# tuna2134/sbv2-api

Measured on NVIDIA B200. Metric: audio-sec/sec, higher is better.
Workload: dtype f16 operands / f32 accumulate on tcgen05 (decoder, flow; text encoder with two-term fp16 splits); f32 elsewhere

## Files before the change

sbv2-api_b200/csrc/flow_attention_tc.cu:

```cuda
#include <cuda_fp16.h>
#include <math_constants.h>

#include "kernels.h"

namespace sbv2 {
namespace {

constexpr int QT = 128, KT = 128, D = 96, DP = D / 8, RP = 16;
constexpr uint32_t TILE_BYTES = DP * KT * 16;
constexpr uint32_t P_BYTES = (KT / 8) * QT * 16;
constexpr uint32_t PREL_BYTES = (RP / 8) * QT * 16;
constexpr uint32_t REL_BYTES = DP * RP * 16;
constexpr int TM_O = 0, TM_SREL = 96, TM_S = 128 , TM_COLS = 512;
constexpr int NKV = 3;
constexpr int NSM_WARPS = 8;

__device__ __forceinline__ uint32_t smem_u32(const void* p) { return (uint32_t)__cvta_generic_to_shared(p); }
__device__ __forceinline__ void mbar_init(uint32_t bar, uint32_t count) {
  asm volatile("mbarrier.init.shared::cta.b64 [%0], %1;" ::"r"(bar), "r"(count));
}
__device__ __forceinline__ void mbar_expect_tx(uint32_t bar, uint32_t bytes) {
  asm volatile("mbarrier.arrive.expect_tx.shared::cta.b64 _, [%0], %1;" ::"r"(bar), "r"(bytes) : "memory");
}
__device__ __forceinline__ void mbar_arrive(uint32_t bar) {
  asm volatile("mbarrier.arrive.shared::cta.b64 _, [%0];" ::"r"(bar) : "memory");
}
__device__ __forceinline__ void mbar_wait(uint32_t bar, uint32_t parity) {
  asm volatile(
      "{\n"
      ".reg .pred P1;\n"
      "LAB_WAIT:\n"
      "mbarrier.try_wait.parity.shared::cta.b64 P1, [%0], %1, %2;\n"
      "@P1 bra DONE;\n"
      "bra LAB_WAIT;\n"
      "DONE:\n"
      "}\n" ::"r"(bar),
      "r"(parity), "r"(0x989680u)
      : "memory");
}
__device__ __forceinline__ void bulk_g2s(uint32_t dst, const void* src, uint32_t bytes, uint32_t bar) {
  asm volatile("cp.async.bulk.shared::cluster.global.mbarrier::complete_tx::bytes [%0], [%1], %2, [%3];" ::"r"(dst), "l"(src),
               "r"(bytes), "r"(bar)
               : "memory");
}
__device__ __forceinline__ void tc_fence_before() { asm volatile("tcgen05.fence::before_thread_sync;" ::: "memory"); }
__device__ __forceinline__ void tc_fence_after() { asm volatile("tcgen05.fence::after_thread_sync;" ::: "memory"); }
__device__ __forceinline__ void tc_commit(uint32_t bar) {
  asm volatile("tcgen05.commit.cta_group::1.mbarrier::arrive::one.shared::cluster.b64 [%0];" ::"r"(bar) : "memory");
}
__device__ __forceinline__ void tc_mma_f16(uint32_t tmem_d, uint64_t adesc, uint64_t bdesc, uint32_t idesc, uint32_t accumulate) {
  asm volatile(
      "{\n"
      ".reg .pred p;\n"
      "setp.ne.b32 p, %4, 0;\n"
      "tcgen05.mma.cta_group::1.kind::f16 [%0], %1, %2, %3, p;\n"
      "}\n" ::"r"(tmem_d),
      "l"(adesc), "l"(bdesc), "r"(idesc), "r"(accumulate)
      : "memory");
}
__device__ __forceinline__ void tc_ld32(uint32_t taddr, uint32_t* v) {
  asm volatile(
      "tcgen05.ld.sync.aligned.32x32b.x32.b32 "
      "{%0,%1,%2,%3,%4,%5,%6,%7,%8,%9,%10,%11,%12,%13,%14,%15,%16,%17,%18,%19,%20,%21,%22,%23,%24,%25,%26,%27,%28,%29,%30,%31}, [%32];"
      : "=r"(v[0]), "=r"(v[1]), "=r"(v[2]), "=r"(v[3]), "=r"(v[4]), "=r"(v[5]), "=r"(v[6]), "=r"(v[7]), "=r"(v[8]), "=r"(v[9]),
        "=r"(v[10]), "=r"(v[11]), "=r"(v[12]), "=r"(v[13]), "=r"(v[14]), "=r"(v[15]), "=r"(v[16]), "=r"(v[17]), "=r"(v[18]),
        "=r"(v[19]), "=r"(v[20]), "=r"(v[21]), "=r"(v[22]), "=r"(v[23]), "=r"(v[24]), "=r"(v[25]), "=r"(v[26]), "=r"(v[27]),
        "=r"(v[28]), "=r"(v[29]), "=r"(v[30]), "=r"(v[31])
      : "r"(taddr)
      : "memory");
}
__device__ __forceinline__ void tc_ld16(uint32_t taddr, uint32_t* v) {
  asm volatile(
      "tcgen05.ld.sync.aligned.32x32b.x16.b32 {%0,%1,%2,%3,%4,%5,%6,%7,%8,%9,%10,%11,%12,%13,%14,%15}, [%16];"
      : "=r"(v[0]), "=r"(v[1]), "=r"(v[2]), "=r"(v[3]), "=r"(v[4]), "=r"(v[5]), "=r"(v[6]), "=r"(v[7]), "=r"(v[8]), "=r"(v[9]),
        "=r"(v[10]), "=r"(v[11]), "=r"(v[12]), "=r"(v[13]), "=r"(v[14]), "=r"(v[15])
      : "r"(taddr)
      : "memory");
}
__device__ __forceinline__ void tc_wait_ld() { asm volatile("tcgen05.wait::ld.sync.aligned;" ::: "memory"); }
__device__ __forceinline__ uint32_t elect_one_sync() {
  uint32_t pred = 0;
  asm volatile(
      "{\n"
      ".reg .b32 %%rx;\n"
      ".reg .pred %%px;\n"
      "elect.sync %%rx|%%px, %1;\n"
      "@%%px mov.s32 %0, 1;\n"
      "}\n"
      : "+r"(pred)
      : "r"(0xffffffffu));
  return pred;
}
__device__ __forceinline__ float ex2_approx(float x) {
  float y;
  asm("ex2.approx.ftz.f32 %0, %1;" : "=f"(y) : "f"(x));
  return y;
}
__device__ __forceinline__ uint64_t make_desc(uint32_t saddr, uint32_t lbo_bytes, uint32_t sbo_bytes) {
  return (uint64_t)((saddr >> 4) & 0x3FFF) | ((uint64_t)((lbo_bytes >> 4) & 0x3FFF) << 16) | ((uint64_t)((sbo_bytes >> 4) & 0x3FFF) << 32) |
         ((uint64_t)1 << 46);
}
constexpr uint32_t idesc_f16(int n, int b_mn_major) {
  return (1u << 4) | ((uint32_t)b_mn_major << 16) | ((uint32_t)(n >> 3) << 17) | ((uint32_t)(128 >> 4) << 24);
}

#define ATRACE(ev, i)                                                                                   \
  do {                                                                                                   \
    if (trace != nullptr && blockIdx.x == 0 && blockIdx.y == 0 && blockIdx.z == 0 && (i) < 64) trace[(i) * 8 + (ev)] = clock64(); \
  } while (0)

__global__ void __launch_bounds__(288, 1) flow_attention_tc_kernel(__half* out, const __half* qkv, const __half* rel_k_p,
                                                                    const __half* rel_v_p, int heads, int window, PlanarSegs s,
                                                                    long long* trace) {
  extern __shared__ __align__(128) uint8_t smem[];
  const int warp = __shfl_sync(0xffffffffu, (int)(threadIdx.x >> 5), 0), lane = threadIdx.x & 31;
  const int b = s.order ? s.order[blockIdx.z] : (int)blockIdx.z, h = blockIdx.y;
  const int len = s.len[b];
  const int q0 = blockIdx.x * QT;
  if (q0 >= len) return;
  const long long pbase = s.pstart[b];
  const int n_kt = (len + KT - 1) / KT;

  const uint32_t sQ = smem_u32(smem);
  const uint32_t sK0 = sQ + TILE_BYTES;
  const uint32_t sV0 = sK0 + NKV * TILE_BYTES;
  const uint32_t sP = sV0 + NKV * TILE_BYTES;
  const uint32_t sPrel = sP + P_BYTES;
  const uint32_t sEk = sPrel + PREL_BYTES;
  const uint32_t sEv = sEk + REL_BYTES;
  const uint32_t sBar = sEv + REL_BYTES;
  const uint32_t bar_q = sBar, bar_kv = sBar + 8 , bar_kvfree = sBar + 40 , bar_s = sBar + 72 ,
                 bar_sfree = sBar + 88 , bar_p = sBar + 104, bar_pfree = sBar + 112, bar_done = sBar + 120;
  const uint32_t tmem_slot = sBar + 128;
  float* ml_x = reinterpret_cast<float*>(smem + (sBar - sQ) + 256);
  volatile uint32_t* tmem_slot_ptr = reinterpret_cast<volatile uint32_t*>(smem + (tmem_slot - sQ));

  if (threadIdx.x == 0) {
    mbar_init(bar_q, 1);
    for (int i = 0; i < NKV; ++i) {
      mbar_init(bar_kv + 8 * i, 1);
      mbar_init(bar_kvfree + 8 * i, 1);
    }
    mbar_init(bar_s, 1);
    mbar_init(bar_s + 8, 1);
    mbar_init(bar_sfree, 32 * NSM_WARPS);
    mbar_init(bar_sfree + 8, 32 * NSM_WARPS);
    mbar_init(bar_p, 32 * NSM_WARPS);
    mbar_init(bar_pfree, 1);
    mbar_init(bar_done, 1);
    asm volatile("fence.mbarrier_init.release.cluster;" ::: "memory");
  }
  if (warp == NSM_WARPS) {
    asm volatile("tcgen05.alloc.cta_group::1.sync.aligned.shared::cta.b32 [%0], %1;" ::"r"(tmem_slot), "r"((uint32_t)TM_COLS) : "memory");
    asm volatile("tcgen05.relinquish_alloc_permit.cta_group::1.sync.aligned;" ::: "memory");
  }
  if (threadIdx.x < 128) {
    const uint4 z = make_uint4(0, 0, 0, 0);
    *reinterpret_cast<uint4*>(smem + (sPrel - sQ) + threadIdx.x * 16) = z;
    *reinterpret_cast<uint4*>(smem + (sPrel - sQ) + QT * 16 + threadIdx.x * 16) = z;
  }
  asm volatile("fence.proxy.async.shared::cta;" ::: "memory");
  tc_fence_before();
  __syncthreads();
  tc_fence_after();
  const uint32_t tmem = *tmem_slot_ptr;
  pdl_launch_dependents();
  pdl_wait();

  const int q_plane0 = h * DP, k_plane0 = heads * DP + h * DP, v_plane0 = 2 * heads * DP + h * DP;
  const int n_tiles_total = 2 * n_kt;

  if (warp == NSM_WARPS) {
    auto load_tile = [&](int i) {
      const int buf = i % NKV;
      const uint32_t par = ((i / NKV) & 1) ^ 1;
      const int kt = i < n_kt ? i : i - n_kt;
      const bool with_v = i >= n_kt;
      const long long row0 = pbase + (long long)kt * KT;
      mbar_wait(bar_kvfree + 8 * buf, par);
      if (lane == 0) mbar_expect_tx(bar_kv + 8 * buf, with_v ? 2 * TILE_BYTES : TILE_BYTES);
      __syncwarp();
      if (lane < DP) {
        bulk_g2s(sK0 + buf * TILE_BYTES + lane * KT * 16, qkv + (size_t)(k_plane0 + lane) * s.plane_stride + row0 * 8, KT * 16,
                 bar_kv + 8 * buf);
      } else if (lane < 2 * DP && with_v) {
        const int pl = lane - DP;
        bulk_g2s(sV0 + buf * TILE_BYTES + pl * KT * 16, qkv + (size_t)(v_plane0 + pl) * s.plane_stride + row0 * 8, KT * 16,
                 bar_kv + 8 * buf);
      }
      __syncwarp();
    };
    if (elect_one_sync()) {
      mbar_expect_tx(bar_q, TILE_BYTES + 2 * REL_BYTES);
      for (int pl = 0; pl < DP; ++pl)
        bulk_g2s(sQ + pl * QT * 16, qkv + (size_t)(q_plane0 + pl) * s.plane_stride + (pbase + q0) * 8, QT * 16, bar_q);
      bulk_g2s(sEk, rel_k_p, REL_BYTES, bar_q);
      bulk_g2s(sEv, rel_v_p, REL_BYTES, bar_q);
    }
    __syncwarp();
    for (int i = 0; i < NKV && i < n_tiles_total; ++i) load_tile(i);
    mbar_wait(bar_q, 0);
    tc_fence_after();
    const uint64_t dq = make_desc(sQ, QT * 16, 128);
    const uint64_t dek = make_desc(sEk, RP * 16, 128);
    const uint64_t dp = make_desc(sP, QT * 16, 128);
    const uint64_t dprel = make_desc(sPrel, QT * 16, 128);
    const uint64_t dev = make_desc(sEv, 128, RP * 16);
    constexpr uint32_t ID_S = idesc_f16(KT, 0), ID_REL = idesc_f16(RP, 0), ID_O = idesc_f16(D, 1);
    if (elect_one_sync()) {
      for (int k = 0; k < D / 16; ++k)
        tc_mma_f16(tmem + TM_SREL, dq + (uint64_t)(k * 2 * QT), dek + (uint64_t)(k * 2 * RP), ID_REL, k > 0 ? 1u : 0u);
    }
    __syncwarp();
    auto issue_s = [&](int i) {
      const int sb = i & 1, kb = i % NKV;
      mbar_wait(bar_kv + 8 * kb, (i / NKV) & 1);
      if (lane == 0) ATRACE(0, i);
      mbar_wait(bar_sfree + 8 * sb, ((i >> 1) & 1) ^ 1);
      tc_fence_after();
      if (lane == 0) ATRACE(1, i);
      const uint64_t dk = make_desc(sK0 + kb * TILE_BYTES, KT * 16, 128);
      if (elect_one_sync()) {
        for (int k = 0; k < D / 16; ++k)
          tc_mma_f16(tmem + TM_S + sb * KT, dq + (uint64_t)(k * 2 * QT), dk + (uint64_t)(k * 2 * KT), ID_S, k > 0 ? 1u : 0u);
        tc_commit(bar_s + 8 * sb);
        if (i < n_kt) tc_commit(bar_kvfree + 8 * kb);
      }
      __syncwarp();
    };
    issue_s(0);
    for (int i = 0; i < n_tiles_total; ++i) {
      const int kb = i % NKV;
      if (i + 1 < n_tiles_total) issue_s(i + 1);
      if (i >= n_kt) {
        const int j = i - n_kt;
        mbar_wait(bar_p, j & 1);
        tc_fence_after();
        if (lane == 0) ATRACE(2, i);
        const uint64_t dv = make_desc(sV0 + kb * TILE_BYTES, 128, KT * 16);
        if (elect_one_sync()) {
          for (int k = 0; k < KT / 16; ++k)
            tc_mma_f16(tmem + TM_O, dp + (uint64_t)(k * 2 * QT), dv + (uint64_t)(k * 16), ID_O, (j > 0 || k > 0) ? 1u : 0u);
          tc_commit(bar_pfree);
          tc_commit(bar_kvfree + 8 * kb);
        }
        __syncwarp();
      }
      if (i + NKV < n_tiles_total) load_tile(i + NKV);
      if (lane == 0) ATRACE(3, i);
    }
    if (elect_one_sync()) {
      tc_mma_f16(tmem + TM_O, dprel, dev, ID_O, 1u);
      tc_commit(bar_done);
    }
    __syncwarp();
  } else {
    const int quarter = warp & 3, half = warp >> 2;
    const int row = quarter * 32 + lane;
    const int qi = q0 + row;
    const uint32_t lane_addr = tmem + ((uint32_t)(quarter * 32) << 16);
    const float c_scale = 1.4426950408889634f / sqrtf((float)D);
    float srel[9];
    {
      mbar_wait(bar_s, 0);
      tc_fence_after();
      uint32_t v[16];
      tc_ld16(lane_addr + TM_SREL, v);
      tc_wait_ld();
#pragma unroll
      for (int r = 0; r < 9; ++r) srel[r] = __uint_as_float(v[r]) * c_scale;
    }
    float m2 = -CUDART_INF_F, l = 0.f, mb = 0.f;
    uint8_t* prow = smem + (sP - sQ) + row * 16;
    uint8_t* prel_row = smem + (sPrel - sQ) + row * 16;
    auto pass_a = [&](const float* x, float c) {
      float mx = x[0];
#pragma unroll
      for (int e = 1; e < 32; ++e) mx = fmaxf(mx, x[e]);
      m2 = fmaxf(m2, mx * c);
    };
    auto pass_b_store = [&](const float* x, float c, int c32, float* pv) {
      float sum = 0.f;
#pragma unroll
      for (int e = 0; e < 32; ++e) {
        pv[e] = ex2_approx(fmaf(x[e], c, -mb));
        sum += pv[e];
      }
      l += sum;
#pragma unroll
      for (int q = 0; q < 4; ++q) {
        uint4 u;
        __half2* uh = reinterpret_cast<__half2*>(&u);
#pragma unroll
        for (int e = 0; e < 4; ++e) uh[e] = __floats2half2_rn(pv[q * 8 + 2 * e], pv[q * 8 + 2 * e + 1]);
        *reinterpret_cast<uint4*>(prow + (size_t)(c32 * 4 + q) * QT * 16) = u;
      }
    };
    for (int i = 0; i < n_tiles_total; ++i) {
      const bool pass_b = i >= n_kt;
      const int kt = pass_b ? i - n_kt : i;
      const int k0 = kt * KT;
      const int buf = i & 1;
      if (i > 0) {
        mbar_wait(bar_s + 8 * buf, (i >> 1) & 1);
        tc_fence_after();
      }
      if (threadIdx.x == 0) ATRACE(4, i);
      if (i == n_kt) {
        ml_x[(half * QT + row) * 2] = m2;
        asm volatile("bar.sync 1, %0;" ::"r"(32 * NSM_WARPS) : "memory");
        mb = fmaxf(m2, ml_x[((half ^ 1) * QT + row) * 2]);
      }
      if (pass_b && kt > 0) mbar_wait(bar_pfree, (kt - 1) & 1);
      if (threadIdx.x == 0) ATRACE(5, i);
#pragma unroll 1
      for (int cc = 0; cc < KT / 64; ++cc) {
        const int c = half * (KT / 64) + cc;
        const int kc0 = k0 + c * 32;
        if (kc0 >= len) {
          if (pass_b) {
            const uint4 z = make_uint4(0, 0, 0, 0);
#pragma unroll
            for (int q = 0; q < 4; ++q) *reinterpret_cast<uint4*>(prow + (size_t)(c * 4 + q) * QT * 16) = z;
          }
          continue;
        }
        uint32_t v[32];
        tc_ld32(lane_addr + TM_S + buf * KT + c * 32, v);
        tc_wait_ld();
        float* x = reinterpret_cast<float*>(v);
        const int j0 = kc0 - qi + 4;
        const bool band = j0 <= 8 && j0 + 31 >= 0;
        const bool tail = kc0 + 32 > len;
        if (!__any_sync(0xffffffffu, band) && !tail) {
          if (!pass_b) {
            pass_a(x, c_scale);
          } else {
            float pv[32];
            pass_b_store(x, c_scale, c, pv);
          }
          continue;
        }
#pragma unroll
        for (int e = 0; e < 32; ++e) {
          const int r = j0 + e;
          float add = 0.f;
#pragma unroll
          for (int rr = 0; rr < 9; ++rr) add = (r == rr) ? srel[rr] : add;
          x[e] = (kc0 + e < len) ? fmaf(x[e], c_scale, add) : -CUDART_INF_F;
        }
        if (!pass_b) {
          pass_a(x, 1.0f);
        } else {
          float pv[32];
          pass_b_store(x, 1.0f, c, pv);
#pragma unroll
          for (int rr = 0; rr < 9; ++rr) {
            const int e = rr - j0;
            float val = 0.f;
#pragma unroll
            for (int ee = 0; ee < 32; ++ee) val = (e == ee) ? pv[ee] : val;
            if (e >= 0 && e < 32) *reinterpret_cast<__half*>(prel_row + (size_t)(rr >> 3) * QT * 16 + (rr & 7) * 2) = __float2half_rn(val);
          }
        }
      }
      if (threadIdx.x == 0) ATRACE(6, i);
      tc_fence_before();
      mbar_arrive(bar_sfree + 8 * buf);
      if (pass_b) {
        asm volatile("fence.proxy.async.shared::cta;" ::: "memory");
        mbar_arrive(bar_p);
      }
    }
    ml_x[(half * QT + row) * 2 + 1] = l;
    asm volatile("bar.sync 1, %0;" ::"r"(32 * NSM_WARPS) : "memory");
    const float inv_l = 1.0f / (l + ml_x[((half ^ 1) * QT + row) * 2 + 1]);
    mbar_wait(bar_done, 0);
    tc_fence_after();
#pragma unroll 1
    for (int c = half * 2; c < (half == 0 ? 2 : D / 32); ++c) {
      uint32_t v[32];
      tc_ld32(lane_addr + TM_O + c * 32, v);
      tc_wait_ld();
      if (qi < len) {
#pragma unroll
        for (int q = 0; q < 4; ++q) {
          uint4 u;
          __half2* uh = reinterpret_cast<__half2*>(&u);
#pragma unroll
          for (int e = 0; e < 4; ++e)
            uh[e] = __floats2half2_rn(__uint_as_float(v[q * 8 + 2 * e]) * inv_l, __uint_as_float(v[q * 8 + 2 * e + 1]) * inv_l);
          *reinterpret_cast<uint4*>(out + (size_t)(h * DP + c * 4 + q) * s.plane_stride + (pbase + qi) * 8) = u;
        }
      }
    }
  }
  tc_fence_before();
  __syncthreads();
  if (warp == NSM_WARPS) {
    asm volatile("tcgen05.dealloc.cta_group::1.sync.aligned.b32 %0, %1;" ::"r"(tmem), "r"((uint32_t)TM_COLS) : "memory");
  }
}

}

std::vector<__half> pack_flow_rel_table(const float* table, int window, int head_dim) {
  const int R = 2 * window + 1;
  if (head_dim != D || R > RP) fail(SBV2_ERR_UNSUPPORTED, "tensor-core attention: head_dim must be 96 and window at most 7");
  std::vector<__half> pk(size_t(DP) * RP * 8, __float2half(0.f));
  for (int r = 0; r < R; ++r)
    for (int d = 0; d < D; ++d) pk[(size_t(d / 8) * RP + r) * 8 + d % 8] = __float2half_rn(table[size_t(r) * D + d]);
  return pk;
}

void launch_flow_attention_tc(const LaunchCtx& ctx, __half* ctx_out, const __half* qkv, const __half* rel_k_p, const __half* rel_v_p,
                              int heads, int head_dim, int window, const PlanarSegs& s, long long* trace) {
  if (s.n <= 0 || s.max_len <= 0) return;
  if (head_dim != D || window != 4) fail(SBV2_ERR_UNSUPPORTED, "tensor-core attention: head_dim must be 96 and window 4");
  const size_t smem = (1 + 2 * NKV) * TILE_BYTES + P_BYTES + PREL_BYTES + 2 * REL_BYTES + 256 + 2 * QT * 2 * 4;
  static PerDeviceOnce attr_once;
  attr_once.run([&] { CUDA_CHECK(cudaFuncSetAttribute(flow_attention_tc_kernel, cudaFuncAttributeMaxDynamicSharedMemorySize, (int)smem)); });
  dim3 grid((s.max_len + QT - 1) / QT, heads, s.n);
  launch_pdl(ctx.pdl, flow_attention_tc_kernel, grid, dim3(32 * (NSM_WARPS + 1)), smem, ctx.stream, ctx_out, qkv, rel_k_p, rel_v_p, heads, window, s,
             trace);
  ctx.count();
}

}

#ifdef SBV2_DEBUG_HOOKS
#include "model.h"
#include "umma_conv.h"
extern "C" int sbv2_debug_attn_trace(int T, int n_utt, int heads, long long* out_trace , float* out_ms) {
  using namespace sbv2;
  return guarded([&] {
    sbv2_model owner;
    owner.device = 0;
    CUDA_CHECK(cudaSetDevice(0));
    CUDA_CHECK(cudaStreamCreateWithFlags(&owner.stream, cudaStreamNonBlocking));
    LaunchCtx ctx = owner.ctx();
    DBuf meta, qkv, out, tr, rel;
    PinnedBuf pin;
    for (DBuf* b : {&meta, &qkv, &out, &tr, &rel}) b->stream = owner.stream;
    std::vector<int> ystart, ylen, muls{1};
    for (int i = 0; i < n_utt; ++i) {
      ystart.push_back(i * T);
      ylen.push_back(T);
    }
    BatchGeom bg = build_geoms(&owner, meta, pin, ystart, ylen, muls);
    const Geom& G = bg.g[0];
    const int C = heads * D;
    qkv.ensure(size_t(G.rows_tot) * 3 * C * 2);
    out.ensure(size_t(G.rows_tot) * C * 2);
    rel.ensure(2 * REL_BYTES);
    tr.ensure(64 * 8 * 8);
    CUDA_CHECK(cudaMemsetAsync(qkv.p, 0x11, size_t(G.rows_tot) * 3 * C * 2, owner.stream));
    CUDA_CHECK(cudaMemsetAsync(rel.p, 0, 2 * REL_BYTES, owner.stream));
    CUDA_CHECK(cudaMemsetAsync(tr.p, 0, 64 * 8 * 8, owner.stream));
    PlanarSegs ps;
    ps.start = bg.d_ystart;
    ps.pstart = G.d_pstart;
    ps.len = G.d_len;
    ps.n = n_utt;
    ps.max_len = T;
    ps.plane_stride = G.rows_tot * 8;
    const __half* rk = rel.as<__half>();
    const __half* rv = rk + REL_BYTES / 2;
    for (int i = 0; i < 2; ++i) launch_flow_attention_tc(ctx, out.as<__half>(), qkv.as<__half>(), rk, rv, heads, D, 4, ps, nullptr);
    cudaEvent_t e0, e1;
    CUDA_CHECK(cudaEventCreate(&e0));
    CUDA_CHECK(cudaEventCreate(&e1));
    CUDA_CHECK(cudaEventRecord(e0, owner.stream));
    for (int i = 0; i < 5; ++i) launch_flow_attention_tc(ctx, out.as<__half>(), qkv.as<__half>(), rk, rv, heads, D, 4, ps, nullptr);
    CUDA_CHECK(cudaEventRecord(e1, owner.stream));
    launch_flow_attention_tc(ctx, out.as<__half>(), qkv.as<__half>(), rk, rv, heads, D, 4, ps, tr.as<long long>());
    CUDA_CHECK(cudaStreamSynchronize(owner.stream));
    float ms = 0.f;
    CUDA_CHECK(cudaEventElapsedTime(&ms, e0, e1));
    if (out_ms) *out_ms = ms / 5.f;
    cudaEventDestroy(e0);
    cudaEventDestroy(e1);
    if (out_trace) CUDA_CHECK(cudaMemcpy(out_trace, tr.p, 64 * 8 * 8, cudaMemcpyDeviceToHost));
  });
}
#endif
```

Baseline: 9317.

## Shrink flow attention smem/TMEM footprint to fit two CTAs per SM

Reworks the K/V pipeline from three combined K+V buffers into two generic tile slots that are filled with K, V, and then the Ev table in a single item sequence. The S accumulator drops from double to single buffering, and Ek is staged in the P region. TMEM allocation is halved to 256 columns and launch bounds allow two CTAs per SM. The S-free barrier now fires right after the last TMEM read, so the next QK^T can start earlier. The aim is to overlap work from two CTAs per SM on large grids; in exchange, per-CTA pipelining depth drops. Small grids launch with a padded shared-memory size so they still get one CTA per SM. A debug timing hook is also added.

```diff
diff --git a/sbv2-api_b200/csrc/flow_attention_tc.cu b/sbv2-api_b200/csrc/flow_attention_tc.cu
--- a/sbv2-api_b200/csrc/flow_attention_tc.cu
+++ b/sbv2-api_b200/csrc/flow_attention_tc.cu
@@ -11,9 +11,15 @@
 constexpr uint32_t P_BYTES = (KT / 8) * QT * 16;
 constexpr uint32_t PREL_BYTES = (RP / 8) * QT * 16;
 constexpr uint32_t REL_BYTES = DP * RP * 16;
-constexpr int TM_O = 0, TM_SREL = 96, TM_S = 128 , TM_COLS = 512;
-constexpr int NKV = 3;
+constexpr int TM_O = 0, TM_SREL = 96, TM_S = 128, TM_COLS = 256;
+constexpr int NSLOT = 2;
 constexpr int NSM_WARPS = 8;
+constexpr uint32_t BAR_BYTES = 256, ML_BYTES = 2 * QT * 2 * 4;
+constexpr uint32_t SMEM_BYTES = (1 + NSLOT) * TILE_BYTES + P_BYTES + PREL_BYTES + BAR_BYTES + ML_BYTES;
+static_assert(2 * (SMEM_BYTES + 1024) <= 228 * 1024, "two CTAs per SM must fit");
+constexpr uint32_t SOLO_SMEM_BYTES = 200 * 1024;
+static_assert(SOLO_SMEM_BYTES + 1024 > 114 * 1024 && SOLO_SMEM_BYTES + 1024 <= 227 * 1024, "one CTA per SM, within the opt-in limit");
+static_assert(REL_BYTES <= P_BYTES && REL_BYTES <= TILE_BYTES, "Ek / Ev are staged in the P region / a tile slot");
 
 __device__ __forceinline__ uint32_t smem_u32(const void* p) { return (uint32_t)__cvta_generic_to_shared(p); }
 __device__ __forceinline__ void mbar_init(uint32_t bar, uint32_t count) {
@@ -109,7 +115,7 @@
     if (trace != nullptr && blockIdx.x == 0 && blockIdx.y == 0 && blockIdx.z == 0 && (i) < 64) trace[(i) * 8 + (ev)] = clock64(); \
   } while (0)
 
-__global__ void __launch_bounds__(288, 1) flow_attention_tc_kernel(__half* out, const __half* qkv, const __half* rel_k_p,
+__global__ void __launch_bounds__(288, 2) flow_attention_tc_kernel(__half* out, const __half* qkv, const __half* rel_k_p,
                                                                     const __half* rel_v_p, int heads, int window, PlanarSegs s,
                                                                     long long* trace) {
   extern __shared__ __align__(128) uint8_t smem[];
@@ -122,29 +128,25 @@
   const int n_kt = (len + KT - 1) / KT;
 
   const uint32_t sQ = smem_u32(smem);
-  const uint32_t sK0 = sQ + TILE_BYTES;
-  const uint32_t sV0 = sK0 + NKV * TILE_BYTES;
-  const uint32_t sP = sV0 + NKV * TILE_BYTES;
+  const uint32_t sR0 = sQ + TILE_BYTES;
+  const uint32_t sP = sR0 + NSLOT * TILE_BYTES;
+  const uint32_t sEk = sP;
   const uint32_t sPrel = sP + P_BYTES;
-  const uint32_t sEk = sPrel + PREL_BYTES;
-  const uint32_t sEv = sEk + REL_BYTES;
-  const uint32_t sBar = sEv + REL_BYTES;
-  const uint32_t bar_q = sBar, bar_kv = sBar + 8 , bar_kvfree = sBar + 40 , bar_s = sBar + 72 ,
-                 bar_sfree = sBar + 88 , bar_p = sBar + 104, bar_pfree = sBar + 112, bar_done = sBar + 120;
-  const uint32_t tmem_slot = sBar + 128;
-  float* ml_x = reinterpret_cast<float*>(smem + (sBar - sQ) + 256);
+  const uint32_t sBar = sPrel + PREL_BYTES;
+  const uint32_t bar_q = sBar, bar_kv = sBar + 8 , bar_kvfree = sBar + 24 , bar_s = sBar + 40,
+                 bar_sfree = sBar + 48, bar_p = sBar + 56, bar_pfree = sBar + 64, bar_done = sBar + 72;
+  const uint32_t tmem_slot = sBar + 80;
+  float* ml_x = reinterpret_cast<float*>(smem + (sBar - sQ) + BAR_BYTES);
   volatile uint32_t* tmem_slot_ptr = reinterpret_cast<volatile uint32_t*>(smem + (tmem_slot - sQ));
 
   if (threadIdx.x == 0) {
     mbar_init(bar_q, 1);
-    for (int i = 0; i < NKV; ++i) {
+    for (int i = 0; i < NSLOT; ++i) {
       mbar_init(bar_kv + 8 * i, 1);
       mbar_init(bar_kvfree + 8 * i, 1);
     }
     mbar_init(bar_s, 1);
-    mbar_init(bar_s + 8, 1);
     mbar_init(bar_sfree, 32 * NSM_WARPS);
-    mbar_init(bar_sfree + 8, 32 * NSM_WARPS);
     mbar_init(bar_p, 32 * NSM_WARPS);
     mbar_init(bar_pfree, 1);
     mbar_init(bar_done, 1);
@@ -171,41 +173,47 @@
   const int n_tiles_total = 2 * n_kt;
 
   if (warp == NSM_WARPS) {
-    auto load_tile = [&](int i) {
-      const int buf = i % NKV;
-      const uint32_t par = ((i / NKV) & 1) ^ 1;
-      const int kt = i < n_kt ? i : i - n_kt;
-      const bool with_v = i >= n_kt;
+    const int n_items = 3 * n_kt + 1, t_ev = 3 * n_kt;
+    auto kitem = [&](int i) { return i < n_kt ? i : 2 * i - n_kt; };
+    int next_item = 0;
+    auto load_item = [&](int t) {
+      const int slot = t % NSLOT;
+      const uint32_t dst = sR0 + slot * TILE_BYTES, bar = bar_kv + 8 * slot;
+      mbar_wait(bar_kvfree + 8 * slot, ((t / NSLOT) & 1) ^ 1);
+      if (t == t_ev) {
+        if (elect_one_sync()) {
+          mbar_expect_tx(bar, REL_BYTES);
+          bulk_g2s(dst, rel_v_p, REL_BYTES, bar);
+        }
+        __syncwarp();
+        return;
+      }
+      const bool is_v = t >= n_kt && ((t - n_kt) & 1);
+      const int kt = t < n_kt ? t : (t - n_kt) >> 1;
       const long long row0 = pbase + (long long)kt * KT;
-      mbar_wait(bar_kvfree + 8 * buf, par);
-      if (lane == 0) mbar_expect_tx(bar_kv + 8 * buf, with_v ? 2 * TILE_BYTES : TILE_BYTES);
+      if (lane == 0) mbar_expect_tx(bar, TILE_BYTES);
       __syncwarp();
-      if (lane < DP) {
-        bulk_g2s(sK0 + buf * TILE_BYTES + lane * KT * 16, qkv + (size_t)(k_plane0 + lane) * s.plane_stride + row0 * 8, KT * 16,
-                 bar_kv + 8 * buf);
-      } else if (lane < 2 * DP && with_v) {
-        const int pl = lane - DP;
-        bulk_g2s(sV0 + buf * TILE_BYTES + pl * KT * 16, qkv + (size_t)(v_plane0 + pl) * s.plane_stride + row0 * 8, KT * 16,
-                 bar_kv + 8 * buf);
-      }
+      if (lane < DP)
+        bulk_g2s(dst + lane * KT * 16, qkv + (size_t)((is_v ? v_plane0 : k_plane0) + lane) * s.plane_stride + row0 * 8, KT * 16, bar);
       __syncwarp();
     };
+    auto load_upto = [&](int last) {
+      for (; next_item <= last && next_item < n_items; ++next_item) load_item(next_item);
+    };
     if (elect_one_sync()) {
-      mbar_expect_tx(bar_q, TILE_BYTES + 2 * REL_BYTES);
+      mbar_expect_tx(bar_q, TILE_BYTES + REL_BYTES);
       for (int pl = 0; pl < DP; ++pl)
         bulk_g2s(sQ + pl * QT * 16, qkv + (size_t)(q_plane0 + pl) * s.plane_stride + (pbase + q0) * 8, QT * 16, bar_q);
       bulk_g2s(sEk, rel_k_p, REL_BYTES, bar_q);
-      bulk_g2s(sEv, rel_v_p, REL_BYTES, bar_q);
     }
     __syncwarp();
-    for (int i = 0; i < NKV && i < n_tiles_total; ++i) load_tile(i);
+    load_upto(NSLOT - 1);
     mbar_wait(bar_q, 0);
     tc_fence_after();
     const uint64_t dq = make_desc(sQ, QT * 16, 128);
     const uint64_t dek = make_desc(sEk, RP * 16, 128);
     const uint64_t dp = make_desc(sP, QT * 16, 128);
     const uint64_t dprel = make_desc(sPrel, QT * 16, 128);
-    const uint64_t dev = make_desc(sEv, 128, RP * 16);
     constexpr uint32_t ID_S = idesc_f16(KT, 0), ID_REL = idesc_f16(RP, 0), ID_O = idesc_f16(D, 1);
     if (elect_one_sync()) {
       for (int k = 0; k < D / 16; ++k)
@@ -213,47 +221,53 @@
     }
     __syncwarp();
     auto issue_s = [&](int i) {
-      const int sb = i & 1, kb = i % NKV;
-      mbar_wait(bar_kv + 8 * kb, (i / NKV) & 1);
+      const int t = kitem(i), slot = t % NSLOT;
+      mbar_wait(bar_kv + 8 * slot, (t / NSLOT) & 1);
       if (lane == 0) ATRACE(0, i);
-      mbar_wait(bar_sfree + 8 * sb, ((i >> 1) & 1) ^ 1);
+      mbar_wait(bar_sfree, (i & 1) ^ 1);
       tc_fence_after();
       if (lane == 0) ATRACE(1, i);
-      const uint64_t dk = make_desc(sK0 + kb * TILE_BYTES, KT * 16, 128);
+      const uint64_t dk = make_desc(sR0 + slot * TILE_BYTES, KT * 16, 128);
       if (elect_one_sync()) {
         for (int k = 0; k < D / 16; ++k)
-          tc_mma_f16(tmem + TM_S + sb * KT, dq + (uint64_t)(k * 2 * QT), dk + (uint64_t)(k * 2 * KT), ID_S, k > 0 ? 1u : 0u);
-        tc_commit(bar_s + 8 * sb);
-        if (i < n_kt) tc_commit(bar_kvfree + 8 * kb);
+          tc_mma_f16(tmem + TM_S, dq + (uint64_t)(k * 2 * QT), dk + (uint64_t)(k * 2 * KT), ID_S, k > 0 ? 1u : 0u);
+        tc_commit(bar_s);
+        tc_commit(bar_kvfree + 8 * slot);
       }
       __syncwarp();
     };
     issue_s(0);
     for (int i = 0; i < n_tiles_total; ++i) {
-      const int kb = i % NKV;
       if (i + 1 < n_tiles_total) issue_s(i + 1);
       if (i >= n_kt) {
-        const int j = i - n_kt;
+        const int j = i - n_kt, t = kitem(i) + 1, slot = t % NSLOT;
         mbar_wait(bar_p, j & 1);
+        mbar_wait(bar_kv + 8 * slot, (t / NSLOT) & 1);
         tc_fence_after();
         if (lane == 0) ATRACE(2, i);
-        const uint64_t dv = make_desc(sV0 + kb * TILE_BYTES, 128, KT * 16);
+        const uint64_t dv = make_desc(sR0 + slot * TILE_BYTES, 128, KT * 16);
         if (elect_one_sync()) {
           for (int k = 0; k < KT / 16; ++k)
             tc_mma_f16(tmem + TM_O, dp + (uint64_t)(k * 2 * QT), dv + (uint64_t)(k * 16), ID_O, (j > 0 || k > 0) ? 1u : 0u);
           tc_commit(bar_pfree);
-          tc_commit(bar_kvfree + 8 * kb);
+          tc_commit(bar_kvfree + 8 * slot);
         }
         __syncwarp();
       }
-      if (i + NKV < n_tiles_total) load_tile(i + NKV);
+      load_upto((i + 1 < n_tiles_total ? kitem(i + 1) : t_ev - 1) + NSLOT);
       if (lane == 0) ATRACE(3, i);
     }
-    if (elect_one_sync()) {
-      tc_mma_f16(tmem + TM_O, dprel, dev, ID_O, 1u);
-      tc_commit(bar_done);
-    }
-    __syncwarp();
+    {
+      const int slot = t_ev % NSLOT;
+      mbar_wait(bar_kv + 8 * slot, (t_ev / NSLOT) & 1);
+      tc_fence_after();
+      const uint64_t dev = make_desc(sR0 + slot * TILE_BYTES, 128, RP * 16);
+      if (elect_one_sync()) {
+        tc_mma_f16(tmem + TM_O, dprel, dev, ID_O, 1u);
+        tc_commit(bar_done);
+      }
+      __syncwarp();
+    }
   } else {
     const int quarter = warp & 3, half = warp >> 2;
     const int row = quarter * 32 + lane;
@@ -300,9 +314,8 @@
       const bool pass_b = i >= n_kt;
       const int kt = pass_b ? i - n_kt : i;
       const int k0 = kt * KT;
-      const int buf = i & 1;
       if (i > 0) {
-        mbar_wait(bar_s + 8 * buf, (i >> 1) & 1);
+        mbar_wait(bar_s, i & 1);
         tc_fence_after();
       }
       if (threadIdx.x == 0) ATRACE(4, i);
@@ -313,6 +326,7 @@
       }
       if (pass_b && kt > 0) mbar_wait(bar_pfree, (kt - 1) & 1);
       if (threadIdx.x == 0) ATRACE(5, i);
+      bool s_read = false;
 #pragma unroll 1
       for (int cc = 0; cc < KT / 64; ++cc) {
         const int c = half * (KT / 64) + cc;
@@ -326,8 +340,13 @@
           continue;
         }
         uint32_t v[32];
-        tc_ld32(lane_addr + TM_S + buf * KT + c * 32, v);
+        tc_ld32(lane_addr + TM_S + c * 32, v);
         tc_wait_ld();
+        if (cc == KT / 64 - 1) {
+          tc_fence_before();
+          mbar_arrive(bar_sfree);
+          s_read = true;
+        }
         float* x = reinterpret_cast<float*>(v);
         const int j0 = kc0 - qi + 4;
         const bool band = j0 <= 8 && j0 + 31 >= 0;
@@ -365,8 +384,10 @@
         }
       }
       if (threadIdx.x == 0) ATRACE(6, i);
-      tc_fence_before();
-      mbar_arrive(bar_sfree + 8 * buf);
+      if (!s_read) {
+        tc_fence_before();
+        mbar_arrive(bar_sfree);
+      }
       if (pass_b) {
         asm volatile("fence.proxy.async.shared::cta;" ::: "memory");
         mbar_arrive(bar_p);
@@ -402,6 +423,16 @@
   }
 }
 
+size_t flow_attention_smem_bytes(const dim3& grid) {
+  static int num_sms = 0;
+  if (num_sms == 0) {
+    int dev = 0;
+    CUDA_CHECK(cudaGetDevice(&dev));
+    CUDA_CHECK(cudaDeviceGetAttribute(&num_sms, cudaDevAttrMultiProcessorCount, dev));
+  }
+  return (long long)grid.x * grid.y * grid.z <= num_sms ? SOLO_SMEM_BYTES : SMEM_BYTES;
+}
+
 }
 
 std::vector<__half> pack_flow_rel_table(const float* table, int window, int head_dim) {
@@ -417,10 +448,13 @@
                               int heads, int head_dim, int window, const PlanarSegs& s, long long* trace) {
   if (s.n <= 0 || s.max_len <= 0) return;
   if (head_dim != D || window != 4) fail(SBV2_ERR_UNSUPPORTED, "tensor-core attention: head_dim must be 96 and window 4");
-  const size_t smem = (1 + 2 * NKV) * TILE_BYTES + P_BYTES + PREL_BYTES + 2 * REL_BYTES + 256 + 2 * QT * 2 * 4;
   static PerDeviceOnce attr_once;
-  attr_once.run([&] { CUDA_CHECK(cudaFuncSetAttribute(flow_attention_tc_kernel, cudaFuncAttributeMaxDynamicSharedMemorySize, (int)smem)); });
+  attr_once.run([&] {
+    CUDA_CHECK(cudaFuncSetAttribute(flow_attention_tc_kernel, cudaFuncAttributeMaxDynamicSharedMemorySize, (int)SOLO_SMEM_BYTES));
+    CUDA_CHECK(cudaFuncSetAttribute(flow_attention_tc_kernel, cudaFuncAttributePreferredSharedMemoryCarveout, cudaSharedmemCarveoutMaxShared));
+  });
   dim3 grid((s.max_len + QT - 1) / QT, heads, s.n);
+  const size_t smem = flow_attention_smem_bytes(grid);
   launch_pdl(ctx.pdl, flow_attention_tc_kernel, grid, dim3(32 * (NSM_WARPS + 1)), smem, ctx.stream, ctx_out, qkv, rel_k_p, rel_v_p, heads, window, s,
              trace);
   ctx.count();
@@ -483,4 +517,82 @@
     if (out_trace) CUDA_CHECK(cudaMemcpy(out_trace, tr.p, 64 * 8 * 8, cudaMemcpyDeviceToHost));
   });
 }
+
+extern "C" int sbv2_debug_flow_attention_time(const int* lens, int n, int heads, int warmup, int iters, float* out_us,
+                                              int* out_ctas_per_sm, int* out_attr) {
+  using namespace sbv2;
+  return guarded([&] {
+    SBV2_REQUIRE(n > 0 && heads > 0 && warmup >= 0 && iters > 0, "bad arguments");
+    sbv2_model owner;
+    owner.device = 0;
+    CUDA_CHECK(cudaSetDevice(0));
+    CUDA_CHECK(cudaStreamCreateWithFlags(&owner.stream, cudaStreamNonBlocking));
+    LaunchCtx ctx = owner.ctx();
+    DBuf meta, qkv, out, rel;
+    PinnedBuf pin;
+    for (DBuf* b : {&meta, &qkv, &out, &rel}) b->stream = owner.stream;
+    std::vector<int> ystart, ylen(lens, lens + n), muls{1};
+    int rows = 0;
+    for (int b = 0; b < n; ++b) {
+      SBV2_REQUIRE(lens[b] >= 1, "utterance lengths must be positive");
+      ystart.push_back(rows);
+      rows += lens[b];
+    }
+    BatchGeom bg = build_geoms(&owner, meta, pin, ystart, ylen, muls);
+    const Geom& G = bg.g[0];
+    const size_t qkv_bytes = size_t(G.rows_tot) * 3 * heads * D * 2;
+    qkv.ensure(qkv_bytes);
+    out.ensure(size_t(G.rows_tot) * heads * D * 2);
+    rel.ensure(2 * REL_BYTES);
+    CUDA_CHECK(cudaMemsetAsync(qkv.p, 0x11, qkv_bytes, owner.stream));
+    CUDA_CHECK(cudaMemsetAsync(rel.p, 0, 2 * REL_BYTES, owner.stream));
+    PlanarSegs ps;
+    ps.start = bg.d_ystart;
+    ps.pstart = G.d_pstart;
+    ps.len = G.d_len;
+    ps.order = bg.d_order;
+    ps.n = n;
+    ps.max_len = G.max_len;
+    ps.plane_stride = G.rows_tot * 8;
+    const __half* rk = rel.as<__half>();
+    const __half* rv = rk + REL_BYTES / 2;
+    auto launch = [&] { launch_flow_attention_tc(ctx, out.as<__half>(), qkv.as<__half>(), rk, rv, heads, D, 4, ps, nullptr); };
+    for (int i = 0; i < std::max(warmup, 1); ++i) launch();
+    cudaEvent_t e0, e1;
+    CUDA_CHECK(cudaEventCreate(&e0));
+    CUDA_CHECK(cudaEventCreate(&e1));
+    CUDA_CHECK(cudaEventRecord(e0, owner.stream));
+    for (int i = 0; i < iters; ++i) launch();
+    CUDA_CHECK(cudaEventRecord(e1, owner.stream));
+    CUDA_CHECK(cudaStreamSynchronize(owner.stream));
+    float ms = 0.f;
+    CUDA_CHECK(cudaEventElapsedTime(&ms, e0, e1));
+    cudaEventDestroy(e0);
+    cudaEventDestroy(e1);
+    if (out_us) *out_us = ms * 1e3f / float(iters);
+    const int launch_smem = (int)flow_attention_smem_bytes(dim3((G.max_len + QT - 1) / QT, heads, n));
+    cudaFuncAttributes fa;
+    CUDA_CHECK(cudaFuncGetAttributes(&fa, flow_attention_tc_kernel));
+    int ctas = 0;
+    CUDA_CHECK(cudaOccupancyMaxActiveBlocksPerMultiprocessor(&ctas, flow_attention_tc_kernel, 32 * (NSM_WARPS + 1), launch_smem));
+    if (out_ctas_per_sm) *out_ctas_per_sm = ctas;
+    if (out_attr) {
+      size_t avail2 = 0;
+      if (cudaOccupancyAvailableDynamicSMemPerBlock(&avail2, flow_attention_tc_kernel, 2, 32 * (NSM_WARPS + 1)) != cudaSuccess) {
+        (void)cudaGetLastError();
+        avail2 = size_t(-1);
+      }
+      int sm_smem = 0, reserved = 0;
+      CUDA_CHECK(cudaDeviceGetAttribute(&sm_smem, cudaDevAttrMaxSharedMemoryPerMultiprocessor, 0));
+      CUDA_CHECK(cudaDeviceGetAttribute(&reserved, cudaDevAttrReservedSharedMemoryPerBlock, 0));
+      out_attr[0] = fa.numRegs;
+      out_attr[1] = launch_smem;
+      out_attr[2] = int(avail2);
+      out_attr[3] = sm_smem;
+      out_attr[4] = reserved;
+      out_attr[5] = fa.preferredShmemCarveout;
+      out_attr[6] = int(fa.sharedSizeBytes);
+    }
+  });
+}
 #endif
```

After: 9432 (median of 6 runs). No clear change (+1.2%).
